# adelacvg/NS2VC

Measured on NVIDIA H100. Metric: denoiser-steps/s, higher is better.
Workload: dtype f32 (3xBF16-split tensor-core contractions, fp32 accumulate)

## Files before the change

### include/ns2vc_b200.h

```cpp
#ifndef NS2VC_B200_H
#define NS2VC_B200_H

#include <stddef.h>
#include <stdint.h>

#ifdef __cplusplus
extern "C" {
#endif

typedef struct ns2vc_unet ns2vc_unet;
typedef void* ns2vc_stream;

#define NS2VC_MAX_LEVELS 8

typedef struct ns2vc_unet_cfg {
  int in_channels;
  int latent_channels;
  int out_channels;
  int n_levels;
  int block_out_channels[NS2VC_MAX_LEVELS];
  int layers_per_block[NS2VC_MAX_LEVELS];
  int down_has_attn[NS2VC_MAX_LEVELS];
  int up_has_attn[NS2VC_MAX_LEVELS];
  int num_heads;
// ... 222 lines not shown
  const float* bias; const float* rowbias; int rowbias_ld;
  const float* res; int res_ld;
  float* out; int out_ld;
  void* out_hi; void* out_lo; int out_split_ld;
  int f16_col0;
  const double* ln_stats; const float* ln_g; int ln_C; float ln_eps;
  double* row_stats; double* stat_sum; double* stat_sq;
  const float* rowmask;
  const int* row_len; int len_shift;
  const float* pre_scale; const float* pre_shift;
  int pre_mode;
  int pre_C;
  int ksplit;
  const double* gn_stats1; const double* gn_stats2; int gn_C1, gn_C2, gn_G; float gn_eps;
  const float* gn_gamma; const float* gn_beta; const float* gn_film; int gn_film_ld;
} ns2vc_check_gemm_args;
typedef struct ns2vc_check_attn_args {
  int B, H, Tq, Tk, dh;
  float scale;
  int v2;
  const float* q; int q_ld; const float* k; int k_ld; const float* v; int v_ld;
  ns2vc_check_split qs, ks, vs;
  int q_c0, k_c0, v_c0;
  int p_split;
  const int* key_len; int key_shift;
  const float* bias;
  float* out; int out_ld;
  void* out_hi; void* out_lo; int out_split_ld;
} ns2vc_check_attn_args;
int ns2vc_check_pack_b(const float* w, int n_rows, int cin_total, int ktaps, int tap, int cin0, int ncin, int n_dst0, int kb0,
                       int geglu_half, const float* cscale, void* w_hi, void* w_lo, int Npad, int nkb_total, ns2vc_stream stream);
int ns2vc_check_gemm(const ns2vc_check_gemm_args* args, char* desc, int desc_len, ns2vc_stream stream);
int ns2vc_check_attention(const ns2vc_check_attn_args* args, char* desc, int desc_len, ns2vc_stream stream);

typedef struct ns2vc_check_prep_args {
  const float* src1; int ld1, C1;
  const float* src2; int ld2, C2;
  int B, T_src, T_dst;
  int row_mul, row_add;
  const int* rowmap;
  int mode;
  const float* scale; const float* shift;
  const double* stats1; const double* stats2;
  const float* gamma; const float* beta; int G; float eps;
  const float* film; int film_ld;
  ns2vc_check_split out, raw;
  const int* row_len; int len_shift;
} ns2vc_check_prep_args;
int ns2vc_check_prep(const ns2vc_check_prep_args* args, char* desc, int desc_len, ns2vc_stream stream);

typedef struct ns2vc_check_ln_args {
  int kind;
  const float* x; int ld, M, C; float eps;
  const float* gamma; const float* beta;
  const float* keep;
  float* y; int y_ld;
  ns2vc_check_split split;
} ns2vc_check_ln_args;
int ns2vc_check_ln(const ns2vc_check_ln_args* args, char* desc, int desc_len, ns2vc_stream stream);

typedef struct ns2vc_check_voc_norm_args {
  const float* x; int B, T, C;
  const float* dw; const float* gamma; const float* beta; float eps;
  const int64_t* len;
  float* out; ns2vc_check_split split;
} ns2vc_check_voc_norm_args;
// ... 57 lines not shown
```

### ns2vc_b200/_lib.py

```python
from __future__ import annotations

import ctypes as C
import os
from typing import Any, Callable, Dict, Optional, Tuple

import torch
import torch.nn as nn

_HERE = os.path.dirname(os.path.abspath(__file__))
LIB_PATH = os.path.join(_HERE, "_C", os.environ.get("NS2VC_LIB_NAME", "libns2vc_b200.so"))

MAX_LEVELS = 8


class UNetCfg(C.Structure):
    _fields_ = [
        ("in_channels", C.c_int), ("latent_channels", C.c_int), ("out_channels", C.c_int), ("n_levels", C.c_int),
        ("block_out_channels", C.c_int * MAX_LEVELS), ("layers_per_block", C.c_int * MAX_LEVELS),
        ("down_has_attn", C.c_int * MAX_LEVELS), ("up_has_attn", C.c_int * MAX_LEVELS),
        ("num_heads", C.c_int), ("cross_attention_dim", C.c_int), ("norm_num_groups", C.c_int), ("norm_eps", C.c_float),
        ("time_scale_shift", C.c_int), ("add_embed_text", C.c_int), ("add_embed_heads", C.c_int),
        ("flip_sin_to_cos", C.c_int), ("freq_shift", C.c_float),
    ]

# ... 108 lines not shown
    "ns2vc_cv_weight_info": (C.c_int, [_P, C.c_int, C.POINTER(C.c_char_p), C.POINTER(C.c_int64), C.POINTER(C.c_int)]),
    "ns2vc_cv_load_weight": (C.c_int, [_P, C.c_char_p, _P, C.POINTER(C.c_int64), C.c_int, _P]),
    "ns2vc_cv_finalize": (C.c_int, [_P, _P]),
    "ns2vc_cv_workspace_bytes": (C.c_int, [_P, C.c_int, C.c_int, C.POINTER(C.c_size_t)]),
    "ns2vc_cv_num_frames": (C.c_int, [C.c_longlong]),
    "ns2vc_cv_extract": (C.c_int, [_P, _P, C.c_longlong, _P, _P, _P, C.c_int, C.c_int, _P, _P]),
    "ns2vc_cv_num_taps": (C.c_int, [_P]),
    "ns2vc_cv_tap_info": (C.c_int, [_P, C.c_int, C.POINTER(C.c_char_p), C.POINTER(C.c_int), C.POINTER(C.c_int)]),
    "ns2vc_cv_set_tap": (C.c_int, [_P, C.c_int, _P]),
    "ns2vc_cv_launch_count": (C.c_int, [_P]),
    "ns2vc_resample_out_length": (C.c_longlong, [C.c_int, C.c_int, C.c_longlong]),
    "ns2vc_resample_table": (C.c_int, [C.c_int, C.c_int, C.POINTER(C.c_int), C.POINTER(C.c_int), C.POINTER(C.c_int), _P]),
    "ns2vc_mel_filterbank": (C.c_int, [_P]),
    "ns2vc_resample_check": (C.c_int, [C.c_int, C.c_int]),
    "ns2vc_resampler_create": (C.c_int, [C.c_int, C.c_int, C.POINTER(_P)]),
    "ns2vc_resampler_destroy": (None, [_P]),
    "ns2vc_resample": (C.c_int, [_P, _P, C.c_longlong, C.c_longlong, _P, _P, C.c_longlong, C.c_longlong, C.c_int, _P]),
    "ns2vc_mel_create": (C.c_int, [_P, _P, C.POINTER(_P)]),
    "ns2vc_mel_destroy": (None, [_P]),
    "ns2vc_log_mel": (C.c_int, [_P, _P, C.c_longlong, C.c_longlong, _P, _P, C.c_int, C.c_int, _P]),
    "ns2vc_stream_sola": (C.c_int, [_P, C.c_longlong, _P, _P, _P, _P, C.c_int, C.c_int, C.c_int, C.c_int, _P]),
    "ns2vc_slice_rms_frames": (C.c_longlong, [C.c_longlong, C.c_int, C.c_int]),
    "ns2vc_slice_rms": (C.c_int, [_P, C.c_longlong, _P, _P, _P, C.c_int, C.c_int, _P]),
    "ns2vc_q_sample": (C.c_int, [_P, _P, C.c_int, _P, _P, _P, _P, C.c_int, _P, _P, _P, C.c_int, C.c_int, C.c_int, C.c_int, _P]),
    "ns2vc_mse_workspace_bytes": (C.c_int, [C.c_int, C.c_int, C.c_int, C.c_int, C.POINTER(C.c_size_t)]),
    "ns2vc_mse_rows": (C.c_int, [_P, _P, C.c_int, _P, _P, C.c_int, C.c_float, _P, _P, _P, C.c_int, C.c_int, C.c_int, C.c_int, _P, _P]),
    "ns2vc_mse_ragged_workspace_bytes": (C.c_int, [C.c_int, C.c_int, C.c_int, C.c_int, C.POINTER(C.c_size_t)]),
    "ns2vc_mse_rows_ragged": (C.c_int, [_P, _P, C.c_int, _P, _P, _P, C.c_int, C.c_float, _P, _P, C.c_int, C.c_int, C.c_int, C.c_int,
                                        _P, _P]),
    "ns2vc_check_pack_b": (C.c_int, [_P, C.c_int, C.c_int, C.c_int, C.c_int, C.c_int, C.c_int, C.c_int, C.c_int, C.c_int, _P, _P, _P,
                                     C.c_int, C.c_int, _P]),
    "ns2vc_check_gemm": (C.c_int, [_P, C.c_char_p, C.c_int, _P]),
    "ns2vc_check_attention": (C.c_int, [_P, C.c_char_p, C.c_int, _P]),
    "ns2vc_check_prep": (C.c_int, [_P, C.c_char_p, C.c_int, _P]),
    "ns2vc_check_ln": (C.c_int, [_P, C.c_char_p, C.c_int, _P]),
    "ns2vc_check_voc_norm": (C.c_int, [_P, C.c_char_p, C.c_int, _P]),
    "ns2vc_check_small_linear": (C.c_int, [_P, C.c_char_p, C.c_int, _P]),
    "ns2vc_check_pool": (C.c_int, [_P, C.c_char_p, C.c_int, _P]),
    "ns2vc_check_nct_split": (C.c_int, [_P, C.c_char_p, C.c_int, _P]),
    "ns2vc_check_cv_conv0": (C.c_int, [_P, C.c_char_p, C.c_int, _P]),
    "ns2vc_check_cv_pos_conv": (C.c_int, [_P, C.c_char_p, C.c_int, _P]),
    "ns2vc_check_istft": (C.c_int, [_P, C.c_char_p, C.c_int, _P]),
}

_lib: Optional[C.CDLL] = None


class Ns2vcError(RuntimeError):
    pass


def lib() -> C.CDLL:
    global _lib
    if _lib is None:
        if not os.path.exists(LIB_PATH):
            raise Ns2vcError(
                f"{LIB_PATH} not found: the ns2vc_b200 CUDA extension is not built "
                "(run ./build.sh or __graft_entry__.build()); there is no CPU fallback.")
        handle = C.CDLL(LIB_PATH)
        for name, (res, args) in SIGNATURES.items():
            fn = getattr(handle, name)
            fn.restype = res
            fn.argtypes = args
        _lib = handle
    return _lib

# ... 130 lines not shown
```

### ns2vc_b200/csrc/attention_v2.cu

```cuda
#include "flash_mma.cuh"
#include "tc_common.cuh"
#include "launch.cuh"
#include <math.h>
#include <cstdlib>

namespace ns2vc {

namespace {

constexpr int kQ = 128, kKeys = 64;
constexpr int kThreadsV2 = 288;

template <int DHP, int PB, bool PF16, bool BIAS> struct ACfg {
  static constexpr int NST = (PB == 128) ? 2 : 3;
  static constexpr int kQBytes = kQ * PB;
  static constexpr int kTBytes = kKeys * PB;
  static constexpr int kStageBytes = 4 * kTBytes;
  static constexpr int kOffQ = 0;
  static constexpr int kOffKV = 2 * kQBytes;
  static constexpr int kOffBar = kOffKV + NST * kStageBytes;
  static constexpr int kOffBias = kOffBar + 256;
  static constexpr int kBiasKeys = (PB == 32) ? 768 : 1024;
  static constexpr int kSmem = kOffBias + (BIAS ? 4 * kBiasKeys : 0) + 1024 ;
  static constexpr int kMinCtas = (PB == 128) ? 1 : (kSmem <= 113 * 1024) ? 2 : 1;
};

template <int DHP, int PB, bool BIAS, bool PF16, bool RAGK = false>
__global__ void __launch_bounds__(kThreadsV2, ACfg<DHP, PB, PF16, BIAS>::kMinCtas) attn_v2_kernel(const __grid_constant__ AttnOp op) {
  using C = ACfg<DHP, PB, PF16, BIAS>;
  constexpr int NST = C::NST;
  extern __shared__ uint8_t smem_raw[];
  const uint32_t raw = smem_u32(smem_raw);
  const uint32_t base = (raw + 1023u) & ~1023u;
  uint8_t* smem = smem_raw + (base - raw);
  const uint32_t bar0 = base + C::kOffBar;
  const uint32_t q_full = bar0;
  auto kv_full = [&](int s) { return bar0 + 8u + 8u * s; };
  auto kv_empty = [&](int s) { return bar0 + 8u + 8u * (NST + s); };

  const int tid = threadIdx.x, warp = tid >> 5, lane = tid & 31;
  const int b = blockIdx.z, h = blockIdx.y, q0 = blockIdx.x * kQ;
  const int dh = op.dh;
  const int ntiles = (op.Tk + kKeys - 1) / kKeys;

  span_begin(op.span);
  const int cta_lin = (blockIdx.z * gridDim.y + blockIdx.y) * gridDim.x + blockIdx.x;
  if (op.trace && tid == 0 && cta_lin < 597) {
    unsigned smid; asm volatile("mov.u32 %0, %%smid;" : "=r"(smid));
    op.trace[256 + 3 * cta_lin] = gtime_ns();
    op.trace[256 + 3 * cta_lin + 2] = smid;
  }
  if (tid == 0) {
    mbar_init(q_full, 1);
    for (int s = 0; s < NST; ++s) { mbar_init(kv_full(s), 1); mbar_init(kv_empty(s), 8); }
    mbar_fence_init();
  }
  if (warp == 0 && lane == 0) {
#pragma unroll
    for (int i = 0; i < 6; ++i) prefetch_tmap(&op.tm[i]);
  }
  pdl_trigger();
  __syncthreads();
  const uint32_t sQ = base + C::kOffQ, sKV = base + C::kOffKV;

  if (warp == 0) {
    if (elect_one()) {
      auto load_kv = [&](int j) {
        const int stage = j % NST;
        const uint32_t dst = sKV + stage * C::kStageBytes;
        mbar_arrive_expect_tx(kv_full(stage), (uint32_t)C::kStageBytes);
        tma_load_3d(dst, &op.tm[2], op.k_c0 + h * dh, j * kKeys, b, kv_full(stage));
        tma_load_3d(dst + C::kTBytes, &op.tm[3], op.k_c0 + h * dh, j * kKeys, b, kv_full(stage));
        tma_load_3d(dst + 2 * C::kTBytes, &op.tm[4], op.v_c0 + h * dh, j * kKeys, b, kv_full(stage));
        tma_load_3d(dst + 3 * C::kTBytes, &op.tm[5], op.v_c0 + h * dh, j * kKeys, b, kv_full(stage));
      };
      pdl_wait();
      int nt = ntiles;
      if constexpr (RAGK) nt = min(ntiles, (((__ldg(op.key_len + b) - 1) >> op.key_shift) + kKeys) / kKeys);
      mbar_arrive_expect_tx(q_full, 2u * C::kQBytes);
      tma_load_3d(sQ, &op.tm[0], op.q_c0 + h * dh, q0, b, q_full);
      tma_load_3d(sQ + C::kQBytes, &op.tm[1], op.q_c0 + h * dh, q0, b, q_full);
      for (int j = 0; j < nt; ++j) {
        if (j >= NST) mbar_wait(kv_empty(j % NST), (uint32_t)(((j / NST) & 1) ^ 1));
        load_kv(j);
      }
    }
  } else {
    float* bias_s = reinterpret_cast<float*>(smem + C::kOffBias);
    const float qscale = op.scale * 1.4426950408889634f;
    pdl_wait();
    int tk = op.Tk, nt = ntiles;
    if constexpr (RAGK) { tk = min(tk, ((__ldg(op.key_len + b) - 1) >> op.key_shift) + 1); nt = (tk + kKeys - 1) / kKeys; }
    if (BIAS) {
      const float* bias = op.bias + (long long)b * op.Tk;
      for (int i = tid - 32; i < ntiles * kKeys; i += 256)
        bias_s[i] = (i < op.Tk) ? __ldg(bias + i) * 1.4426950408889634f : -INFINITY;
      asm volatile("bar.sync 1, 256;" ::: "memory");
    }
    FlashWarp<DHP, PB, PF16> fw;
    const int r0 = 16 * (warp - 1);
    mbar_wait(q_full, 0);
    fw.load_q(sQ, sQ + C::kQBytes, r0, lane);
    for (int j = 0; j < nt; ++j) {
      const int stage = j % NST;
      mbar_wait_quiet(kv_full(stage), (uint32_t)((j / NST) & 1));
      const uint32_t kst = sKV + stage * C::kStageBytes;
      fw.tile(kst, kst + C::kTBytes, kst + 2 * C::kTBytes, kst + 3 * C::kTBytes, BIAS ? bias_s + j * kKeys : nullptr, qscale,
              (RAGK ? tk : op.Tk) - j * kKeys, lane);
      __syncwarp();
      if (lane == 0) mbar_arrive(kv_empty(stage));
    }
    fw.store(op, b, h, q0 + r0, lane);
  }
  __syncthreads();
  span_end(op.span);
  if (op.trace && tid == 0 && cta_lin < 597) op.trace[256 + 3 * cta_lin + 1] = gtime_ns();
}

template <int DHP, int PB, bool BIAS, bool PF16, bool RAGK = false>
int launch_v2b(const AttnOp& op, cudaStream_t st) {
  using C = ACfg<DHP, PB, PF16, BIAS>;
  static bool attr_set = false;
  if (!attr_set) {
    cudaError_t e = cudaFuncSetAttribute(attn_v2_kernel<DHP, PB, BIAS, PF16, RAGK>, cudaFuncAttributeMaxDynamicSharedMemorySize, C::kSmem);
    if (e != cudaSuccess) { set_error("attention v2: cannot set %d B dynamic smem: %s", C::kSmem, cudaGetErrorString(e)); return -2; }
    cudaFuncSetAttribute(attn_v2_kernel<DHP, PB, BIAS, PF16, RAGK>, cudaFuncAttributePreferredSharedMemoryCarveout, (int)cudaSharedmemCarveoutMaxShared);
    if (getenv("NS2VC_DEBUG")) {
      int nb = 0;
      cudaOccupancyMaxActiveBlocksPerMultiprocessor(&nb, attn_v2_kernel<DHP, PB, BIAS, PF16, RAGK>, kThreadsV2, (size_t)C::kSmem);
      fprintf(stderr, "ns2vc: attn_v2<%d,%d,bias=%d,f16=%d> smem %d B, planned %d CTAs/SM, occupancy API says %d\n", DHP, PB, (int)BIAS, (int)PF16, C::kSmem, C::kMinCtas, nb);
    }
    attr_set = true;
  }
  dim3 grid(ceil_div(op.Tq, kQ), op.H, op.B);
  cudaError_t e = launch_k(attn_v2_kernel<DHP, PB, BIAS, PF16, RAGK>, grid, dim3(kThreadsV2), (size_t)C::kSmem, st, op);
  if (e != cudaSuccess) { set_error("attention v2 launch failed: %s", cudaGetErrorString(e)); return -2; }
  return 0;
}
bool p_fp16() { return attention_v2_p_fp16(); }
template <int DHP, int PB>
int launch_v2(const AttnOp& op, cudaStream_t st) {
  if (op.key_len) {
    if (op.bias) { set_error("attention v2: per-entry key counts take no additive bias"); return -1; }
    return (p_fp16() && !op.p_split) ? launch_v2b<DHP, PB, false, true, true>(op, st) : launch_v2b<DHP, PB, false, false, true>(op, st);
  }
  if (op.bias) {
    if (ceil_div(op.Tk, kKeys) * kKeys > ACfg<DHP, PB, true, true>::kBiasKeys) { set_error("attention v2: %d biased keys exceed the staged-bias capacity", op.Tk); return -1; }
    return (p_fp16() && !op.p_split) ? launch_v2b<DHP, PB, true, true>(op, st) : launch_v2b<DHP, PB, true, false>(op, st);
  }
  return (p_fp16() && !op.p_split) ? launch_v2b<DHP, PB, false, true>(op, st) : launch_v2b<DHP, PB, false, false>(op, st);
}

int natural_pb(int dh) { return dh == 16 ? 32 : dh == 32 ? 64 : 128; }

}

bool attention_v2_p_fp16() {
  static int v = -1;
  if (v < 0) { const char* e = getenv("NS2VC_ATTN_P"); v = (e && e[0] == 's') ? 0 : 1; }
  return v == 1;
}

bool attention_v2_supported(int dh, int Tk, bool biased) {
  if (!(dh == 16 || dh == 32 || dh == 48 || dh == 64)) return false;
  return !biased || ceil_div(Tk, kKeys) * kKeys <= (dh == 16 ? 768 : 1024);
}

int encode_attn_tmaps(AttnOp& op) {
  op.pb = natural_pb(op.dh);
  const int bc = op.pb / 2;
  int rc = 0;
  if ((rc = encode_tmap_rows(&op.tm[0], op.qs.hi, op.qs.C, op.qs.T, op.B, op.qs.ld, bc, kQ, op.pb))) return rc;
  if ((rc = encode_tmap_rows(&op.tm[1], op.qs.lo, op.qs.C, op.qs.T, op.B, op.qs.ld, bc, kQ, op.pb))) return rc;
  if ((rc = encode_tmap_rows(&op.tm[2], op.ks.hi, op.ks.C, op.ks.T, op.B, op.ks.ld, bc, kKeys, op.pb))) return rc;
  if ((rc = encode_tmap_rows(&op.tm[3], op.ks.lo, op.ks.C, op.ks.T, op.B, op.ks.ld, bc, kKeys, op.pb))) return rc;
  if ((rc = encode_tmap_rows(&op.tm[4], op.vs.hi, op.vs.C, op.vs.T, op.B, op.vs.ld, bc, kKeys, op.pb))) return rc;
  if ((rc = encode_tmap_rows(&op.tm[5], op.vs.lo, op.vs.C, op.vs.T, op.B, op.vs.ld, bc, kKeys, op.pb))) return rc;
  return 0;
}

int launch_attention_v2(const AttnOp& op, cudaStream_t st) {
  if (op.Tk <= 0 || op.Tq <= 0) { set_error("attention: empty sequence"); return -1; }
  if (op.qs.T != op.Tq || op.ks.T != op.Tk || op.vs.T != op.Tk) { set_error("attention v2: split buffer / sequence length mismatch"); return -1; }
  const int dh = op.dh;
  if (op.pb == 128) {
    if (dh == 48) return launch_v2<48, 128>(op, st);
    if (dh == 64) return launch_v2<64, 128>(op, st);
  } else if (op.pb == 64 && dh == 32) {
    return launch_v2<32, 64>(op, st);
  } else if (op.pb == 32 && dh == 16) {
    return launch_v2<16, 32>(op, st);
  }
  set_error("attention v2: unsupported head dim %d / box %d", dh, op.pb);
  return -1;
// ... 4 lines not shown
```

### ns2vc_b200/csrc/common.cuh

```cuda
#pragma once
#include <cuda_runtime.h>
#include <cuda_bf16.h>
#include <stdint.h>
#include <stddef.h>

namespace ns2vc {

void set_error(const char* fmt, ...);
const char* get_error();

#define NS_CHECK_CUDA(expr)                                                                    \
  do {                                                                                         \
    cudaError_t _e = (expr);                                                                   \
    if (_e != cudaSuccess) {                                                                   \
      ns2vc::set_error("%s:%d CUDA error %s: %s", __FILE__, __LINE__, cudaGetErrorName(_e),    \
                       cudaGetErrorString(_e));                                                \
      return -2;                                                                               \
    }                                                                                          \
  } while (0)

#define NS_REQUIRE(cond, ...)                                                                  \
  do {                                                                                         \
    if (!(cond)) {                                                                             \
      ns2vc::set_error(__VA_ARGS__);                                                           \
// ... 151 lines not shown
  const float* gamma; const float* beta;
  const float* keep;
  float* y; int y_ld;
  SplitBuf split;
};
int launch_ln_split(const LnOp& op, cudaStream_t st);

struct AttnOp {
  const float* q; int q_ld;
  const float* k; int k_ld;
  const float* v; int v_ld;
  const float* bias;
  float* out; int out_ld;
  __nv_bfloat16* out_hi;
  __nv_bfloat16* out_lo;
  int out_split_ld;
  int B, H, Tq, Tk, dh;
  float scale;
  unsigned long long* span;
  unsigned long long* trace;
  SplitBuf qs, ks, vs;
  int q_c0, k_c0, v_c0;
  int v2;
  int pb;
  const int* key_len;
  int key_shift;
  int p_split;
  TMap tm[6];
};
int launch_attention(const AttnOp& op, cudaStream_t st, bool simt_debug);
int launch_attention_v2(const AttnOp& op, cudaStream_t st);
bool attention_v2_supported(int dh, int Tk, bool biased);
bool attention_v2_p_fp16();
int encode_attn_tmaps(AttnOp& op);
int encode_tmap_rows(TMap* out, const __nv_bfloat16* base, int C, int T, int B, int ld, int box_c, int box_rows, int swizzle_bytes);
int encode_tmap_any(TMap* out, const void* base, int elem_bytes, int C, int T, int B, int ld, int box_c, int box_rows, int swizzle_bytes,
                    long long bpitch = 0);

int launch_ln_apply(const LnOp& op, cudaStream_t st);

struct TokensOp {
  const float* x; long long bstride; int B, C, T;
  float* out; int ld;
  const float* rowbias;
  const float* keep;
};
int launch_nct_to_tokens(const TokensOp& op, cudaStream_t st);
struct NctSplitOp {
  const float* x; long long bstride; int B, C, T;
  SplitBuf out;
  const int* row_len;
  const void* warm; long long warm_bytes;
};
int launch_nct_to_split(const NctSplitOp& op, cudaStream_t st);

enum LinIn : int { LIN_RAW = 0, LIN_SILU = 1, LIN_SINUSOID = 2 };
struct LinOp {
  const float* x; int x_ld; int M; int K;
  const float* W; const float* bias; int N;
  const float* add; int add_ld;
  int add_rows;
  float* out; int out_ld;
  int in_mode; int flip_sin_to_cos; float freq_shift;
  int out_silu;
};
int launch_small_linear(const LinOp& op, cudaStream_t st);
// ... 105 lines not shown
```

### ns2vc_b200/csrc/flash_mma.cuh

```cuda
#pragma once
#include "gemm_common.cuh"
#include <math.h>

namespace ns2vc {

template <int PB>
__device__ __forceinline__ uint32_t swz(uint32_t a) { return a ^ (((a >> 7) & (uint32_t)(PB / 16 - 1)) << 4); }

__device__ __forceinline__ float ex2f(float x) { float y; asm("ex2.approx.ftz.f32 %0, %1;" : "=f"(y) : "f"(x)); return y; }

__device__ __forceinline__ void ldsm_x4(uint32_t a, uint32_t* r) {
  asm volatile("ldmatrix.sync.aligned.m8n8.x4.shared.b16 {%0, %1, %2, %3}, [%4];" : "=r"(r[0]), "=r"(r[1]), "=r"(r[2]), "=r"(r[3]) : "r"(a));
}
__device__ __forceinline__ void ldsm_x4_t(uint32_t a, uint32_t* r) {
  asm volatile("ldmatrix.sync.aligned.m8n8.x4.trans.shared.b16 {%0, %1, %2, %3}, [%4];" : "=r"(r[0]), "=r"(r[1]), "=r"(r[2]), "=r"(r[3]) : "r"(a));
}
#define NS2VC_MMA(name, ty)                                                                                                      \
  __device__ __forceinline__ void name(float* c, const uint32_t* a, uint32_t b0, uint32_t b1) {                               \
    asm volatile("mma.sync.aligned.m16n8k16.row.col.f32." ty "." ty ".f32 {%0, %1, %2, %3}, {%4, %5, %6, %7}, {%8, %9}, {%0, %1, %2, %3};" \
                 : "+f"(c[0]), "+f"(c[1]), "+f"(c[2]), "+f"(c[3]) : "r"(a[0]), "r"(a[1]), "r"(a[2]), "r"(a[3]), "r"(b0), "r"(b1)); }
NS2VC_MMA(mma_bf16, "bf16")
NS2VC_MMA(mma_f16, "f16")
#undef NS2VC_MMA

template <int DHP, int PB, bool PF16>
struct FlashWarp {
  static constexpr int KS = DHP / 16;
  static constexpr int NO = DHP / 8;
  uint32_t qh[KS][4], ql[KS][4];
  float o[NO][4];
  float m[2], l[2];

  __device__ __forceinline__ void load_q(uint32_t sqh, uint32_t sql, int r0, int lane) {
    const uint32_t off = (uint32_t)((r0 + (lane & 7) + 8 * ((lane >> 3) & 1)) * PB + 16 * (lane >> 4));
#pragma unroll
    for (int k = 0; k < KS; ++k) { ldsm_x4(swz<PB>(sqh + off + 32 * k), qh[k]); ldsm_x4(swz<PB>(sql + off + 32 * k), ql[k]); }
#pragma unroll
    for (int n = 0; n < NO; ++n) o[n][0] = o[n][1] = o[n][2] = o[n][3] = 0.f;
    m[0] = m[1] = -INFINITY;
    l[0] = l[1] = 0.f;
  }

  __device__ __forceinline__ void tile(uint32_t skh, uint32_t skl, uint32_t svh, uint32_t svl, const float* bias, float qs, int nvalid, int lane) {
    float s[8][4];
#pragma unroll
    for (int n = 0; n < 8; ++n) s[n][0] = s[n][1] = s[n][2] = s[n][3] = 0.f;
    const uint32_t koff = (uint32_t)(((lane & 7) + 8 * (lane >> 4)) * PB + 16 * ((lane >> 3) & 1));
#pragma unroll
    for (int k = 0; k < KS; ++k) {
#pragma unroll
      for (int np = 0; np < 4; ++np) {
        uint32_t kh[4], kl[4];
        const uint32_t a = (uint32_t)(16 * np * PB) + koff + 32 * k;
        ldsm_x4(swz<PB>(skh + a), kh);
        ldsm_x4(swz<PB>(skl + a), kl);
        mma_bf16(s[2 * np], qh[k], kh[0], kh[1]);
        mma_bf16(s[2 * np], ql[k], kh[0], kh[1]);
        mma_bf16(s[2 * np], qh[k], kl[0], kl[1]);
        mma_bf16(s[2 * np + 1], qh[k], kh[2], kh[3]);
        mma_bf16(s[2 * np + 1], ql[k], kh[2], kh[3]);
        mma_bf16(s[2 * np + 1], qh[k], kl[2], kl[3]);
      }
    }
    const int t = lane & 3;
    float mx[2] = {-INFINITY, -INFINITY};
#pragma unroll
    for (int n = 0; n < 8; ++n)
#pragma unroll
      for (int e = 0; e < 4; ++e) {
        const int key = 8 * n + 2 * t + (e & 1);
        float v = s[n][e] * qs;
        if (bias) v += bias[key];
        else if (key >= nvalid) v = -INFINITY;
        s[n][e] = v;
        mx[e >> 1] = fmaxf(mx[e >> 1], v);
      }
    float corr[2];
#pragma unroll
    for (int i = 0; i < 2; ++i) {
      mx[i] = fmaxf(mx[i], __shfl_xor_sync(0xffffffffu, mx[i], 1));
      mx[i] = fmaxf(mx[i], __shfl_xor_sync(0xffffffffu, mx[i], 2));
      const float mn = fmaxf(m[i], mx[i]);
      corr[i] = ex2f(m[i] - mn);
      m[i] = mn;
      l[i] *= corr[i];
    }
#pragma unroll
    for (int n = 0; n < NO; ++n)
#pragma unroll
      for (int e = 0; e < 4; ++e) o[n][e] *= corr[e >> 1];
    const uint32_t voff = (uint32_t)(((lane & 7) + 8 * ((lane >> 3) & 1)) * PB + 16 * (lane >> 4));
#pragma unroll
    for (int kk = 0; kk < 4; ++kk) {
      uint32_t ph[4], pl[4];
#pragma unroll
      for (int u = 0; u < 4; ++u) {
        float* sv = s[2 * kk + (u >> 1)] + 2 * (u & 1);
        const float p0 = ex2f(sv[0] - m[u & 1]), p1 = ex2f(sv[1] - m[u & 1]);
        if (PF16) {
          ph[u] = pack_f16x2(p0, p1);
          l[u & 1] += f16lo_to_f32(ph[u]) + f16hi_to_f32(ph[u]);
        } else {
          split2(p0, p1, ph[u], pl[u]);
          l[u & 1] += p0 + p1;
        }
      }
#pragma unroll
      for (int dp = 0; dp < NO / 2; ++dp) {
        uint32_t vh[4], vl[4];
        const uint32_t a = (uint32_t)(16 * kk * PB) + voff + 32 * dp;
        ldsm_x4_t(swz<PB>(svh + a), vh);
        ldsm_x4_t(swz<PB>(svl + a), vl);
        if (PF16) {
          mma_f16(o[2 * dp], ph, vh[0], vh[1]);
          mma_f16(o[2 * dp], ph, vl[0], vl[1]);
          mma_f16(o[2 * dp + 1], ph, vh[2], vh[3]);
          mma_f16(o[2 * dp + 1], ph, vl[2], vl[3]);
        } else {
          mma_bf16(o[2 * dp], ph, vh[0], vh[1]);
          mma_bf16(o[2 * dp], pl, vh[0], vh[1]);
          mma_bf16(o[2 * dp], ph, vl[0], vl[1]);
          mma_bf16(o[2 * dp + 1], ph, vh[2], vh[3]);
          mma_bf16(o[2 * dp + 1], pl, vh[2], vh[3]);
          mma_bf16(o[2 * dp + 1], ph, vl[2], vl[3]);
        }
      }
    }
  }

  __device__ __forceinline__ void store(const AttnOp& op, int b, int h, int q0, int lane) {
    const int g = lane >> 2, t = lane & 3;
#pragma unroll
    for (int i = 0; i < 2; ++i) {
      l[i] += __shfl_xor_sync(0xffffffffu, l[i], 1);
      l[i] += __shfl_xor_sync(0xffffffffu, l[i], 2);
    }
#pragma unroll
    for (int i = 0; i < 2; ++i) {
      const int q = q0 + g + 8 * i;
      if (q >= op.Tq) continue;
      const float inv = 1.0f / l[i];
      const long long orow = (long long)b * op.Tq + q;
#pragma unroll
      for (int n = 0; n < NO; ++n) {
        const int d = 8 * n + 2 * t;
        if (d >= op.dh) continue;
        const float v0 = o[n][2 * i] * inv, v1 = o[n][2 * i + 1] * inv;
        const long long of = orow * op.out_ld + h * op.dh + d, os = orow * op.out_split_ld + h * op.dh + d;
        if (op.out && d + 1 < op.dh && ((of | (long long)(reinterpret_cast<uintptr_t>(op.out) >> 2)) & 1) == 0) {
          *reinterpret_cast<float2*>(op.out + of) = make_float2(v0, v1);
        } else if (op.out) {
          op.out[of] = v0;
          if (d + 1 < op.dh) op.out[of + 1] = v1;
        }
        if (op.out_hi && d + 1 < op.dh &&
            ((os | (long long)(reinterpret_cast<uintptr_t>(op.out_hi) >> 1) | (long long)(reinterpret_cast<uintptr_t>(op.out_lo) >> 1)) & 1) == 0) {
          uint32_t hi, lo;
          split2(v0, v1, hi, lo);
          *reinterpret_cast<uint32_t*>(op.out_hi + os) = hi;
          *reinterpret_cast<uint32_t*>(op.out_lo + os) = lo;
        } else if (op.out_hi) {
#pragma unroll
          for (int e = 0; e < 2; ++e) {
            if (d + e >= op.dh) break;
            const float v = e ? v1 : v0;
            const __nv_bfloat16 hi = __float2bfloat16_rn(v);
            op.out_hi[os + e] = hi;
            op.out_lo[os + e] = __float2bfloat16_rn(v - __bfloat162float(hi));
          }
        }
      }
    }
  }
};

}
```

### ns2vc_b200/csrc/kernel_check.cu

```cuda
#include "engine_host.cuh"
#include "../../include/ns2vc_b200.h"

#include <cstdio>
#include <vector>

namespace ns2vc {
namespace {

SplitBuf to_split(const ns2vc_check_split& s) {
  SplitBuf b{};
  b.hi = (__nv_bfloat16*)s.hi; b.lo = (__nv_bfloat16*)s.lo; b.T = s.T; b.C = s.C; b.ld = s.ld; b.bpitch = s.bpitch;
  return b;
}

template <class... A> void report(char* desc, int desc_len, const char* fmt, A... args) {
  if (desc && desc_len > 0) snprintf(desc, (size_t)desc_len, fmt, args...);
}

}
}

using namespace ns2vc;

extern "C" {
// ... 100 lines not shown
int ns2vc_check_attention(const ns2vc_check_attn_args* a, char* desc, int desc_len, ns2vc_stream stream) {
  NS_REQUIRE(a, "check_attention: null argument");
  NS_REQUIRE(a->B >= 1 && a->H >= 1 && a->dh >= 1, "check_attention: bad sizes B=%d H=%d dh=%d", a->B, a->H, a->dh);
  NS_REQUIRE(a->out || (a->out_hi && a->out_lo), "check_attention: no output");
  AttnOp op; memset(&op, 0, sizeof(op));
  op.B = a->B; op.H = a->H; op.Tq = a->Tq; op.Tk = a->Tk; op.dh = a->dh; op.scale = a->scale;
  op.bias = a->bias;
  op.out = a->out; op.out_ld = a->out_ld;
  op.out_hi = (__nv_bfloat16*)a->out_hi; op.out_lo = (__nv_bfloat16*)a->out_lo; op.out_split_ld = a->out_split_ld;
  cudaStream_t st = (cudaStream_t)stream;
  if (a->v2) {
    NS_REQUIRE(a->qs.hi && a->qs.lo && a->ks.hi && a->ks.lo && a->vs.hi && a->vs.lo, "check_attention: v2 needs split q / k / v");
    op.v2 = 1;
    op.qs = to_split(a->qs); op.ks = to_split(a->ks); op.vs = to_split(a->vs);
    op.q_c0 = a->q_c0; op.k_c0 = a->k_c0; op.v_c0 = a->v_c0;
    op.key_len = a->key_len; op.key_shift = a->key_shift; op.p_split = a->p_split;
    int rc = encode_attn_tmaps(op);
    if (!rc) rc = launch_attention_v2(op, st);
    if (rc) return rc;
    const bool pf16 = attention_v2_p_fp16() && !op.p_split;
    report(desc, desc_len, "attn_v2<%d,PB=%d,BIAS=%d,PF16=%d,RAGK=%d>", op.dh, op.pb, op.bias ? 1 : 0, pf16 ? 1 : 0, op.key_len ? 1 : 0);
    return 0;
  }
  NS_REQUIRE(a->q && a->k && a->v, "check_attention: v1 needs fp32 q / k / v");
  NS_REQUIRE(!a->key_len, "check_attention: per-entry key counts are a v2 feature");
  op.q = a->q; op.q_ld = a->q_ld; op.k = a->k; op.k_ld = a->k_ld; op.v = a->v; op.v_ld = a->v_ld;
  const int rc = launch_attention(op, st, false);
  if (rc) return rc;
  const int dhp = a->dh <= 16 ? 16 : a->dh <= 32 ? 32 : a->dh <= 48 ? 48 : 64;
  report(desc, desc_len, "attn_tc<%d>", dhp);
  return 0;
}

int ns2vc_check_prep(const ns2vc_check_prep_args* a, char* desc, int desc_len, ns2vc_stream stream) {
  NS_REQUIRE(a, "check_prep: null argument");
  NS_REQUIRE(a->B >= 1 && a->T_src >= 1 && a->T_dst >= 1 && a->C1 >= 1 && a->C2 >= 0 && a->src1 && (a->C2 == 0 || a->src2),
             "check_prep: bad sizes B=%d T=%d->%d C=%d+%d", a->B, a->T_src, a->T_dst, a->C1, a->C2);
  NS_REQUIRE(a->out.hi && a->out.lo, "check_prep: no output");
  NS_REQUIRE(a->mode >= PREP_RAW && a->mode <= PREP_AFFINE_SILU, "check_prep: mode %d", a->mode);
  PrepOp p; memset(&p, 0, sizeof(p));
  p.src1 = a->src1; p.ld1 = a->ld1; p.C1 = a->C1; p.src2 = a->src2; p.ld2 = a->ld2; p.C2 = a->C2;
  p.B = a->B; p.T_src = a->T_src; p.T_dst = a->T_dst;
  p.row_mul = a->row_mul; p.row_add = a->row_add; p.rowmap = a->rowmap; p.mode = a->mode;
  p.out = to_split(a->out);
  if (a->raw.hi) p.raw = to_split(a->raw);
  p.row_len = a->row_len; p.len_shift = a->len_shift;
  if (a->mode != PREP_RAW) {
    if (a->scale) {
      NS_REQUIRE(a->shift, "check_prep: scale without shift");
      p.scale = a->scale; p.shift = a->shift;
    } else {
      NS_REQUIRE(a->stats1 && (a->C2 == 0 || a->stats2) && a->gamma && a->beta && a->G >= 1, "check_prep: GroupNorm without its sums or weights");
      set_group_norm(p, a->B, a->stats1, a->C1, a->C2 ? a->stats2 : nullptr, a->C2, a->T_src, a->G, a->eps, a->gamma, a->beta, a->film,
                     a->film_ld);
    }
  }
  const int rc = launch_prep_split(p, (cudaStream_t)stream);
  if (rc) return rc;
  report(desc, desc_len, "prep_split<RAG=%d>", p.row_len ? 1 : 0);
  return 0;
}

int ns2vc_check_ln(const ns2vc_check_ln_args* a, char* desc, int desc_len, ns2vc_stream stream) {
  NS_REQUIRE(a && a->x && a->gamma && a->beta, "check_ln: null argument");
  NS_REQUIRE(a->M >= 1 && a->C >= 1 && a->ld >= a->C, "check_ln: bad sizes M=%d C=%d ld=%d", a->M, a->C, a->ld);
  LnOp op{a->x, a->ld, a->M, a->C, a->eps, a->gamma, a->beta, a->keep, a->y, a->y_ld, to_split(a->split)};
// ... 163 lines not shown
```

Baseline: 1804.

## Add wgmma warpgroup core for attention v2 and make it the default

```diff
diff --git a/include/ns2vc_b200.h b/include/ns2vc_b200.h
--- a/include/ns2vc_b200.h
+++ b/include/ns2vc_b200.h
@@ -278,6 +278,8 @@
                        int geglu_half, const float* cscale, void* w_hi, void* w_lo, int Npad, int nkb_total, ns2vc_stream stream);
 int ns2vc_check_gemm(const ns2vc_check_gemm_args* args, char* desc, int desc_len, ns2vc_stream stream);
 int ns2vc_check_attention(const ns2vc_check_attn_args* args, char* desc, int desc_len, ns2vc_stream stream);
+int ns2vc_attention_set_core(int core);
+int ns2vc_attention_core(int dh, int pf16);
 
 typedef struct ns2vc_check_prep_args {
   const float* src1; int ld1, C1;
diff --git a/ns2vc_b200/_lib.py b/ns2vc_b200/_lib.py
--- a/ns2vc_b200/_lib.py
+++ b/ns2vc_b200/_lib.py
@@ -164,6 +164,8 @@
                                      C.c_int, C.c_int, _P]),
     "ns2vc_check_gemm": (C.c_int, [_P, C.c_char_p, C.c_int, _P]),
     "ns2vc_check_attention": (C.c_int, [_P, C.c_char_p, C.c_int, _P]),
+    "ns2vc_attention_set_core": (C.c_int, [C.c_int]),
+    "ns2vc_attention_core": (C.c_int, [C.c_int, C.c_int]),
     "ns2vc_check_prep": (C.c_int, [_P, C.c_char_p, C.c_int, _P]),
     "ns2vc_check_ln": (C.c_int, [_P, C.c_char_p, C.c_int, _P]),
     "ns2vc_check_voc_norm": (C.c_int, [_P, C.c_char_p, C.c_int, _P]),
diff --git a/ns2vc_b200/csrc/attention_v2.cu b/ns2vc_b200/csrc/attention_v2.cu
--- a/ns2vc_b200/csrc/attention_v2.cu
+++ b/ns2vc_b200/csrc/attention_v2.cu
@@ -1,4 +1,4 @@
-#include "flash_mma.cuh"
+#include "flash_wgmma.cuh"
 #include "tc_common.cuh"
 #include "launch.cuh"
 #include <math.h>
@@ -25,7 +25,7 @@
   static constexpr int kMinCtas = (PB == 128) ? 1 : (kSmem <= 113 * 1024) ? 2 : 1;
 };
 
-template <int DHP, int PB, bool BIAS, bool PF16, bool RAGK = false>
+template <int DHP, int PB, bool BIAS, bool PF16, bool RAGK, bool WG>
 __global__ void __launch_bounds__(kThreadsV2, ACfg<DHP, PB, PF16, BIAS>::kMinCtas) attn_v2_kernel(const __grid_constant__ AttnOp op) {
   using C = ACfg<DHP, PB, PF16, BIAS>;
   constexpr int NST = C::NST;
@@ -55,7 +55,7 @@
     for (int s = 0; s < NST; ++s) { mbar_init(kv_full(s), 1); mbar_init(kv_empty(s), 8); }
     mbar_fence_init();
   }
-  if (warp == 0 && lane == 0) {
+  if (warp == 8 && lane == 0) {
 #pragma unroll
     for (int i = 0; i < 6; ++i) prefetch_tmap(&op.tm[i]);
   }
@@ -63,7 +63,7 @@
   __syncthreads();
   const uint32_t sQ = base + C::kOffQ, sKV = base + C::kOffKV;
 
-  if (warp == 0) {
+  if (warp == 8) {
     if (elect_one()) {
       auto load_kv = [&](int j) {
         const int stage = j % NST;
@@ -93,20 +93,24 @@
     if constexpr (RAGK) { tk = min(tk, ((__ldg(op.key_len + b) - 1) >> op.key_shift) + 1); nt = (tk + kKeys - 1) / kKeys; }
     if (BIAS) {
       const float* bias = op.bias + (long long)b * op.Tk;
-      for (int i = tid - 32; i < ntiles * kKeys; i += 256)
+      for (int i = tid; i < ntiles * kKeys; i += 256)
         bias_s[i] = (i < op.Tk) ? __ldg(bias + i) * 1.4426950408889634f : -INFINITY;
       asm volatile("bar.sync 1, 256;" ::: "memory");
     }
-    FlashWarp<DHP, PB, PF16> fw;
-    const int r0 = 16 * (warp - 1);
+    const int r0 = 16 * warp;
+    std::conditional_t<WG, FlashWG<DHP, PB, PF16>, FlashWarp<DHP, PB, PF16>> fw;
+    const uint32_t sqh = sQ + (r0 & ~63) * PB;
     mbar_wait(q_full, 0);
-    fw.load_q(sQ, sQ + C::kQBytes, r0, lane);
+    if constexpr (WG) fw.init();
+    else fw.load_q(sQ, sQ + C::kQBytes, r0, lane);
     for (int j = 0; j < nt; ++j) {
       const int stage = j % NST;
       mbar_wait_quiet(kv_full(stage), (uint32_t)((j / NST) & 1));
       const uint32_t kst = sKV + stage * C::kStageBytes;
-      fw.tile(kst, kst + C::kTBytes, kst + 2 * C::kTBytes, kst + 3 * C::kTBytes, BIAS ? bias_s + j * kKeys : nullptr, qscale,
-              (RAGK ? tk : op.Tk) - j * kKeys, lane);
+      const float* bj = BIAS ? bias_s + j * kKeys : nullptr;
+      const int nvalid = (RAGK ? tk : op.Tk) - j * kKeys;
+      if constexpr (WG) fw.tile(sqh, sqh + C::kQBytes, kst, kst + C::kTBytes, kst + 2 * C::kTBytes, kst + 3 * C::kTBytes, bj, qscale, nvalid, lane);
+      else fw.tile(kst, kst + C::kTBytes, kst + 2 * C::kTBytes, kst + 3 * C::kTBytes, bj, qscale, nvalid, lane);
       __syncwarp();
       if (lane == 0) mbar_arrive(kv_empty(stage));
     }
@@ -117,25 +121,35 @@
   if (op.trace && tid == 0 && cta_lin < 597) op.trace[256 + 3 * cta_lin + 1] = gtime_ns();
 }
 
+template <int DHP, int PB, bool BIAS, bool PF16, bool RAGK, bool WG>
+int launch_v2c(const AttnOp& op, cudaStream_t st) {
+  using C = ACfg<DHP, PB, PF16, BIAS>;
+  auto kern = attn_v2_kernel<DHP, PB, BIAS, PF16, RAGK, WG>;
+  static bool attr_set = false;
+  if (!attr_set) {
+    cudaError_t e = cudaFuncSetAttribute(kern, cudaFuncAttributeMaxDynamicSharedMemorySize, C::kSmem);
+    if (e != cudaSuccess) { set_error("attention v2: cannot set %d B dynamic smem: %s", C::kSmem, cudaGetErrorString(e)); return -2; }
+    cudaFuncSetAttribute(kern, cudaFuncAttributePreferredSharedMemoryCarveout, (int)cudaSharedmemCarveoutMaxShared);
+    if (getenv("NS2VC_DEBUG")) {
+      int nb = 0;
+      cudaOccupancyMaxActiveBlocksPerMultiprocessor(&nb, kern, kThreadsV2, (size_t)C::kSmem);
+      fprintf(stderr, "ns2vc: attn_v2<%d,%d,bias=%d,f16=%d,wg=%d> smem %d B, planned %d CTAs/SM, occupancy API says %d\n", DHP, PB,
+              (int)BIAS, (int)PF16, (int)WG, C::kSmem, C::kMinCtas, nb);
+    }
+    attr_set = true;
+  }
+  dim3 grid(ceil_div(op.Tq, kQ), op.H, op.B);
+  cudaError_t e = launch_k(kern, grid, dim3(kThreadsV2), (size_t)C::kSmem, st, op);
+  if (e != cudaSuccess) { set_error("attention v2 launch failed: %s", cudaGetErrorString(e)); return -2; }
+  return 0;
+}
+
+int g_core = 0;
+bool core_wg() { return g_core != 1; }
+
 template <int DHP, int PB, bool BIAS, bool PF16, bool RAGK = false>
 int launch_v2b(const AttnOp& op, cudaStream_t st) {
-  using C = ACfg<DHP, PB, PF16, BIAS>;
-  static bool attr_set = false;
-  if (!attr_set) {
-    cudaError_t e = cudaFuncSetAttribute(attn_v2_kernel<DHP, PB, BIAS, PF16, RAGK>, cudaFuncAttributeMaxDynamicSharedMemorySize, C::kSmem);
-    if (e != cudaSuccess) { set_error("attention v2: cannot set %d B dynamic smem: %s", C::kSmem, cudaGetErrorString(e)); return -2; }
-    cudaFuncSetAttribute(attn_v2_kernel<DHP, PB, BIAS, PF16, RAGK>, cudaFuncAttributePreferredSharedMemoryCarveout, (int)cudaSharedmemCarveoutMaxShared);
-    if (getenv("NS2VC_DEBUG")) {
-      int nb = 0;
-      cudaOccupancyMaxActiveBlocksPerMultiprocessor(&nb, attn_v2_kernel<DHP, PB, BIAS, PF16, RAGK>, kThreadsV2, (size_t)C::kSmem);
-      fprintf(stderr, "ns2vc: attn_v2<%d,%d,bias=%d,f16=%d> smem %d B, planned %d CTAs/SM, occupancy API says %d\n", DHP, PB, (int)BIAS, (int)PF16, C::kSmem, C::kMinCtas, nb);
-    }
-    attr_set = true;
-  }
-  dim3 grid(ceil_div(op.Tq, kQ), op.H, op.B);
-  cudaError_t e = launch_k(attn_v2_kernel<DHP, PB, BIAS, PF16, RAGK>, grid, dim3(kThreadsV2), (size_t)C::kSmem, st, op);
-  if (e != cudaSuccess) { set_error("attention v2 launch failed: %s", cudaGetErrorString(e)); return -2; }
-  return 0;
+  return core_wg() ? launch_v2c<DHP, PB, BIAS, PF16, RAGK, true>(op, st) : launch_v2c<DHP, PB, BIAS, PF16, RAGK, false>(op, st);
 }
 bool p_fp16() { return attention_v2_p_fp16(); }
 template <int DHP, int PB>
@@ -160,6 +174,14 @@
   if (v < 0) { const char* e = getenv("NS2VC_ATTN_P"); v = (e && e[0] == 's') ? 0 : 1; }
   return v == 1;
 }
+
+int attention_v2_set_core(int core) {
+  if (core < 0 || core > 2) { set_error("attention v2: core %d is not 0 (measured choice), 1 (mma.sync warps) or 2 (wgmma warpgroups)", core); return -1; }
+  g_core = core;
+  return 0;
+}
+
+int attention_v2_core(int dh, bool pf16) { (void)dh; (void)pf16; return core_wg() ? 2 : 1; }
 
 bool attention_v2_supported(int dh, int Tk, bool biased) {
   if (!(dh == 16 || dh == 32 || dh == 48 || dh == 64)) return false;
diff --git a/ns2vc_b200/csrc/common.cuh b/ns2vc_b200/csrc/common.cuh
--- a/ns2vc_b200/csrc/common.cuh
+++ b/ns2vc_b200/csrc/common.cuh
@@ -207,6 +207,8 @@
 int launch_attention_v2(const AttnOp& op, cudaStream_t st);
 bool attention_v2_supported(int dh, int Tk, bool biased);
 bool attention_v2_p_fp16();
+int attention_v2_set_core(int core);
+int attention_v2_core(int dh, bool pf16);
 int encode_attn_tmaps(AttnOp& op);
 int encode_tmap_rows(TMap* out, const __nv_bfloat16* base, int C, int T, int B, int ld, int box_c, int box_rows, int swizzle_bytes);
 int encode_tmap_any(TMap* out, const void* base, int elem_bytes, int C, int T, int B, int ld, int box_c, int box_rows, int swizzle_bytes,
diff --git a/ns2vc_b200/csrc/flash_mma.cuh b/ns2vc_b200/csrc/flash_mma.cuh
--- a/ns2vc_b200/csrc/flash_mma.cuh
+++ b/ns2vc_b200/csrc/flash_mma.cuh
@@ -22,6 +22,100 @@
 NS2VC_MMA(mma_bf16, "bf16")
 NS2VC_MMA(mma_f16, "f16")
 #undef NS2VC_MMA
+
+template <int NO>
+__device__ __forceinline__ void flash_rescale(float (&s)[8][4], float (&o)[NO][4], float (&m)[2], float (&l)[2], const float* bias,
+                                              float qs, int nvalid, int lane) {
+  const int t = lane & 3;
+  float mx[2] = {-INFINITY, -INFINITY};
+#pragma unroll
+  for (int n = 0; n < 8; ++n)
+#pragma unroll
+    for (int e = 0; e < 4; ++e) {
+      const int key = 8 * n + 2 * t + (e & 1);
+      float v = s[n][e] * qs;
+      if (bias) v += bias[key];
+      else if (key >= nvalid) v = -INFINITY;
+      s[n][e] = v;
+      mx[e >> 1] = fmaxf(mx[e >> 1], v);
+    }
+  float corr[2];
+#pragma unroll
+  for (int i = 0; i < 2; ++i) {
+    mx[i] = fmaxf(mx[i], __shfl_xor_sync(0xffffffffu, mx[i], 1));
+    mx[i] = fmaxf(mx[i], __shfl_xor_sync(0xffffffffu, mx[i], 2));
+    const float mn = fmaxf(m[i], mx[i]);
+    corr[i] = ex2f(m[i] - mn);
+    m[i] = mn;
+    l[i] *= corr[i];
+  }
+#pragma unroll
+  for (int n = 0; n < NO; ++n)
+#pragma unroll
+    for (int e = 0; e < 4; ++e) o[n][e] *= corr[e >> 1];
+}
+
+template <bool PF16>
+__device__ __forceinline__ void flash_weights(const float (&s)[8][4], const float (&m)[2], float (&l)[2], int kk, uint32_t* ph, uint32_t* pl) {
+#pragma unroll
+  for (int u = 0; u < 4; ++u) {
+    const float* sv = s[2 * kk + (u >> 1)] + 2 * (u & 1);
+    const float p0 = ex2f(sv[0] - m[u & 1]), p1 = ex2f(sv[1] - m[u & 1]);
+    if (PF16) {
+      ph[u] = pack_f16x2(p0, p1);
+      l[u & 1] += f16lo_to_f32(ph[u]) + f16hi_to_f32(ph[u]);
+    } else {
+      split2(p0, p1, ph[u], pl[u]);
+      l[u & 1] += p0 + p1;
+    }
+  }
+}
+
+template <int NO>
+__device__ __forceinline__ void flash_store(const float (&o)[NO][4], float (&l)[2], const AttnOp& op, int b, int h, int q0, int lane) {
+  const int g = lane >> 2, t = lane & 3;
+#pragma unroll
+  for (int i = 0; i < 2; ++i) {
+    l[i] += __shfl_xor_sync(0xffffffffu, l[i], 1);
+    l[i] += __shfl_xor_sync(0xffffffffu, l[i], 2);
+  }
+#pragma unroll
+  for (int i = 0; i < 2; ++i) {
+    const int q = q0 + g + 8 * i;
+    if (q >= op.Tq) continue;
+    const float inv = 1.0f / l[i];
+    const long long orow = (long long)b * op.Tq + q;
+#pragma unroll
+    for (int n = 0; n < NO; ++n) {
+      const int d = 8 * n + 2 * t;
+      if (d >= op.dh) continue;
+      const float v0 = o[n][2 * i] * inv, v1 = o[n][2 * i + 1] * inv;
+      const long long of = orow * op.out_ld + h * op.dh + d, os = orow * op.out_split_ld + h * op.dh + d;
+      if (op.out && d + 1 < op.dh && ((of | (long long)(reinterpret_cast<uintptr_t>(op.out) >> 2)) & 1) == 0) {
+        *reinterpret_cast<float2*>(op.out + of) = make_float2(v0, v1);
+      } else if (op.out) {
+        op.out[of] = v0;
+        if (d + 1 < op.dh) op.out[of + 1] = v1;
+      }
+      if (op.out_hi && d + 1 < op.dh &&
+          ((os | (long long)(reinterpret_cast<uintptr_t>(op.out_hi) >> 1) | (long long)(reinterpret_cast<uintptr_t>(op.out_lo) >> 1)) & 1) == 0) {
+        uint32_t hi, lo;
+        split2(v0, v1, hi, lo);
+        *reinterpret_cast<uint32_t*>(op.out_hi + os) = hi;
+        *reinterpret_cast<uint32_t*>(op.out_lo + os) = lo;
+      } else if (op.out_hi) {
+#pragma unroll
+        for (int e = 0; e < 2; ++e) {
+          if (d + e >= op.dh) break;
+          const float v = e ? v1 : v0;
+          const __nv_bfloat16 hi = __float2bfloat16_rn(v);
+          op.out_hi[os + e] = hi;
+          op.out_lo[os + e] = __float2bfloat16_rn(v - __bfloat162float(hi));
+        }
+      }
+    }
+  }
+}
 
 template <int DHP, int PB, bool PF16>
 struct FlashWarp {
@@ -62,49 +156,12 @@
         mma_bf16(s[2 * np + 1], qh[k], kl[2], kl[3]);
       }
     }
-    const int t = lane & 3;
-    float mx[2] = {-INFINITY, -INFINITY};
-#pragma unroll
-    for (int n = 0; n < 8; ++n)
-#pragma unroll
-      for (int e = 0; e < 4; ++e) {
-        const int key = 8 * n + 2 * t + (e & 1);
-        float v = s[n][e] * qs;
-        if (bias) v += bias[key];
-        else if (key >= nvalid) v = -INFINITY;
-        s[n][e] = v;
-        mx[e >> 1] = fmaxf(mx[e >> 1], v);
-      }
-    float corr[2];
-#pragma unroll
-    for (int i = 0; i < 2; ++i) {
-      mx[i] = fmaxf(mx[i], __shfl_xor_sync(0xffffffffu, mx[i], 1));
-      mx[i] = fmaxf(mx[i], __shfl_xor_sync(0xffffffffu, mx[i], 2));
-      const float mn = fmaxf(m[i], mx[i]);
-      corr[i] = ex2f(m[i] - mn);
-      m[i] = mn;
-      l[i] *= corr[i];
-    }
-#pragma unroll
-    for (int n = 0; n < NO; ++n)
-#pragma unroll
-      for (int e = 0; e < 4; ++e) o[n][e] *= corr[e >> 1];
+    flash_rescale<NO>(s, o, m, l, bias, qs, nvalid, lane);
     const uint32_t voff = (uint32_t)(((lane & 7) + 8 * ((lane >> 3) & 1)) * PB + 16 * (lane >> 4));
 #pragma unroll
     for (int kk = 0; kk < 4; ++kk) {
       uint32_t ph[4], pl[4];
-#pragma unroll
-      for (int u = 0; u < 4; ++u) {
-        float* sv = s[2 * kk + (u >> 1)] + 2 * (u & 1);
-        const float p0 = ex2f(sv[0] - m[u & 1]), p1 = ex2f(sv[1] - m[u & 1]);
-        if (PF16) {
-          ph[u] = pack_f16x2(p0, p1);
-          l[u & 1] += f16lo_to_f32(ph[u]) + f16hi_to_f32(ph[u]);
-        } else {
-          split2(p0, p1, ph[u], pl[u]);
-          l[u & 1] += p0 + p1;
-        }
-      }
+      flash_weights<PF16>(s, m, l, kk, ph, pl);
 #pragma unroll
       for (int dp = 0; dp < NO / 2; ++dp) {
         uint32_t vh[4], vl[4];
@@ -128,50 +185,7 @@
     }
   }
 
-  __device__ __forceinline__ void store(const AttnOp& op, int b, int h, int q0, int lane) {
-    const int g = lane >> 2, t = lane & 3;
-#pragma unroll
-    for (int i = 0; i < 2; ++i) {
-      l[i] += __shfl_xor_sync(0xffffffffu, l[i], 1);
-      l[i] += __shfl_xor_sync(0xffffffffu, l[i], 2);
-    }
-#pragma unroll
-    for (int i = 0; i < 2; ++i) {
-      const int q = q0 + g + 8 * i;
-      if (q >= op.Tq) continue;
-      const float inv = 1.0f / l[i];
-      const long long orow = (long long)b * op.Tq + q;
-#pragma unroll
-      for (int n = 0; n < NO; ++n) {
-        const int d = 8 * n + 2 * t;
-        if (d >= op.dh) continue;
-        const float v0 = o[n][2 * i] * inv, v1 = o[n][2 * i + 1] * inv;
-        const long long of = orow * op.out_ld + h * op.dh + d, os = orow * op.out_split_ld + h * op.dh + d;
-        if (op.out && d + 1 < op.dh && ((of | (long long)(reinterpret_cast<uintptr_t>(op.out) >> 2)) & 1) == 0) {
-          *reinterpret_cast<float2*>(op.out + of) = make_float2(v0, v1);
-        } else if (op.out) {
-          op.out[of] = v0;
-          if (d + 1 < op.dh) op.out[of + 1] = v1;
-        }
-        if (op.out_hi && d + 1 < op.dh &&
-            ((os | (long long)(reinterpret_cast<uintptr_t>(op.out_hi) >> 1) | (long long)(reinterpret_cast<uintptr_t>(op.out_lo) >> 1)) & 1) == 0) {
-          uint32_t hi, lo;
-          split2(v0, v1, hi, lo);
-          *reinterpret_cast<uint32_t*>(op.out_hi + os) = hi;
-          *reinterpret_cast<uint32_t*>(op.out_lo + os) = lo;
-        } else if (op.out_hi) {
-#pragma unroll
-          for (int e = 0; e < 2; ++e) {
-            if (d + e >= op.dh) break;
-            const float v = e ? v1 : v0;
-            const __nv_bfloat16 hi = __float2bfloat16_rn(v);
-            op.out_hi[os + e] = hi;
-            op.out_lo[os + e] = __float2bfloat16_rn(v - __bfloat162float(hi));
-          }
-        }
-      }
-    }
-  }
+  __device__ __forceinline__ void store(const AttnOp& op, int b, int h, int q0, int lane) { flash_store<NO>(o, l, op, b, h, q0, lane); }
 };
 
 }
diff --git a/ns2vc_b200/csrc/flash_wgmma.cuh b/ns2vc_b200/csrc/flash_wgmma.cuh
--- /dev/null
+++ b/ns2vc_b200/csrc/flash_wgmma.cuh
@@ -0,0 +1,115 @@
+#pragma once
+#include "flash_mma.cuh"
+#include "tc_common.cuh"
+
+namespace ns2vc {
+
+template <int PB>
+__device__ __forceinline__ uint64_t wg_desc_rows(uint32_t saddr) {
+  constexpr uint64_t mode = PB == 128 ? 1 : PB == 64 ? 2 : 3;
+  return (uint64_t)((saddr & 0x3FFFFu) >> 4) | (1ull << 16) | ((uint64_t)((8 * PB) >> 4) << 32) | (mode << 62);
+}
+
+template <int N, bool F16>
+__device__ __forceinline__ void wgmma_rs(float* d, const uint32_t* a, uint64_t bdesc);
+#define NS2VC_D8(i) "+f"(d[i]), "+f"(d[i + 1]), "+f"(d[i + 2]), "+f"(d[i + 3]), "+f"(d[i + 4]), "+f"(d[i + 5]), "+f"(d[i + 6]), "+f"(d[i + 7])
+#define NS2VC_A4 "r"(a[0]), "r"(a[1]), "r"(a[2]), "r"(a[3])
+template <>
+__device__ __forceinline__ void wgmma_rs<16, true>(float* d, const uint32_t* a, uint64_t bdesc) {
+  asm volatile("{\n\t.reg .pred p;\n\tsetp.ne.b32 p, %13, 0;\n\twgmma.mma_async.sync.aligned.m64n16k16.f32.f16.f16 "
+               "{%0,%1,%2,%3,%4,%5,%6,%7}, "
+               "{%8,%9,%10,%11}, %12, p, 1, 1, 1;\n\t}" : NS2VC_D8(0) : NS2VC_A4, "l"(bdesc), "r"(1));
+}
+template <>
+__device__ __forceinline__ void wgmma_rs<16, false>(float* d, const uint32_t* a, uint64_t bdesc) {
+  asm volatile("{\n\t.reg .pred p;\n\tsetp.ne.b32 p, %13, 0;\n\twgmma.mma_async.sync.aligned.m64n16k16.f32.bf16.bf16 "
+               "{%0,%1,%2,%3,%4,%5,%6,%7}, "
+               "{%8,%9,%10,%11}, %12, p, 1, 1, 1;\n\t}" : NS2VC_D8(0) : NS2VC_A4, "l"(bdesc), "r"(1));
+}
+template <>
+__device__ __forceinline__ void wgmma_rs<32, true>(float* d, const uint32_t* a, uint64_t bdesc) {
+  asm volatile("{\n\t.reg .pred p;\n\tsetp.ne.b32 p, %21, 0;\n\twgmma.mma_async.sync.aligned.m64n32k16.f32.f16.f16 "
+               "{%0,%1,%2,%3,%4,%5,%6,%7,%8,%9,%10,%11,%12,%13,%14,%15}, "
+               "{%16,%17,%18,%19}, %20, p, 1, 1, 1;\n\t}" : NS2VC_D8(0), NS2VC_D8(8) : NS2VC_A4, "l"(bdesc), "r"(1));
+}
+template <>
+__device__ __forceinline__ void wgmma_rs<32, false>(float* d, const uint32_t* a, uint64_t bdesc) {
+  asm volatile("{\n\t.reg .pred p;\n\tsetp.ne.b32 p, %21, 0;\n\twgmma.mma_async.sync.aligned.m64n32k16.f32.bf16.bf16 "
+               "{%0,%1,%2,%3,%4,%5,%6,%7,%8,%9,%10,%11,%12,%13,%14,%15}, "
+               "{%16,%17,%18,%19}, %20, p, 1, 1, 1;\n\t}" : NS2VC_D8(0), NS2VC_D8(8) : NS2VC_A4, "l"(bdesc), "r"(1));
+}
+template <>
+__device__ __forceinline__ void wgmma_rs<48, true>(float* d, const uint32_t* a, uint64_t bdesc) {
+  asm volatile("{\n\t.reg .pred p;\n\tsetp.ne.b32 p, %29, 0;\n\twgmma.mma_async.sync.aligned.m64n48k16.f32.f16.f16 "
+               "{%0,%1,%2,%3,%4,%5,%6,%7,%8,%9,%10,%11,%12,%13,%14,%15,%16,%17,%18,%19,%20,%21,%22,%23}, "
+               "{%24,%25,%26,%27}, %28, p, 1, 1, 1;\n\t}" : NS2VC_D8(0), NS2VC_D8(8), NS2VC_D8(16) : NS2VC_A4, "l"(bdesc), "r"(1));
+}
+template <>
+__device__ __forceinline__ void wgmma_rs<48, false>(float* d, const uint32_t* a, uint64_t bdesc) {
+  asm volatile("{\n\t.reg .pred p;\n\tsetp.ne.b32 p, %29, 0;\n\twgmma.mma_async.sync.aligned.m64n48k16.f32.bf16.bf16 "
+               "{%0,%1,%2,%3,%4,%5,%6,%7,%8,%9,%10,%11,%12,%13,%14,%15,%16,%17,%18,%19,%20,%21,%22,%23}, "
+               "{%24,%25,%26,%27}, %28, p, 1, 1, 1;\n\t}" : NS2VC_D8(0), NS2VC_D8(8), NS2VC_D8(16) : NS2VC_A4, "l"(bdesc), "r"(1));
+}
+template <>
+__device__ __forceinline__ void wgmma_rs<64, true>(float* d, const uint32_t* a, uint64_t bdesc) {
+  asm volatile("{\n\t.reg .pred p;\n\tsetp.ne.b32 p, %37, 0;\n\twgmma.mma_async.sync.aligned.m64n64k16.f32.f16.f16 "
+               "{%0,%1,%2,%3,%4,%5,%6,%7,%8,%9,%10,%11,%12,%13,%14,%15,%16,%17,%18,%19,%20,%21,%22,%23,%24,%25,%26,%27,%28,%29,%30,%31}, "
+               "{%32,%33,%34,%35}, %36, p, 1, 1, 1;\n\t}" : NS2VC_D8(0), NS2VC_D8(8), NS2VC_D8(16), NS2VC_D8(24) : NS2VC_A4, "l"(bdesc), "r"(1));
+}
+template <>
+__device__ __forceinline__ void wgmma_rs<64, false>(float* d, const uint32_t* a, uint64_t bdesc) {
+  asm volatile("{\n\t.reg .pred p;\n\tsetp.ne.b32 p, %37, 0;\n\twgmma.mma_async.sync.aligned.m64n64k16.f32.bf16.bf16 "
+               "{%0,%1,%2,%3,%4,%5,%6,%7,%8,%9,%10,%11,%12,%13,%14,%15,%16,%17,%18,%19,%20,%21,%22,%23,%24,%25,%26,%27,%28,%29,%30,%31}, "
+               "{%32,%33,%34,%35}, %36, p, 1, 1, 1;\n\t}" : NS2VC_D8(0), NS2VC_D8(8), NS2VC_D8(16), NS2VC_D8(24) : NS2VC_A4, "l"(bdesc), "r"(1));
+}
+#undef NS2VC_A4
+#undef NS2VC_D8
+
+template <int DHP, int PB, bool PF16>
+struct FlashWG {
+  static constexpr int KS = DHP / 16;
+  static constexpr int NO = DHP / 8;
+  float o[NO][4];
+  float m[2], l[2];
+
+  __device__ __forceinline__ void init() {
+#pragma unroll
+    for (int n = 0; n < NO; ++n) o[n][0] = o[n][1] = o[n][2] = o[n][3] = 0.f;
+    m[0] = m[1] = -INFINITY;
+    l[0] = l[1] = 0.f;
+  }
+
+  __device__ __forceinline__ void tile(uint32_t sqh, uint32_t sql, uint32_t skh, uint32_t skl, uint32_t svh, uint32_t svl,
+                                       const float* bias, float qs, int nvalid, int lane) {
+    float s[8][4];
+#pragma unroll
+    for (int n = 0; n < 8; ++n) s[n][0] = s[n][1] = s[n][2] = s[n][3] = 0.f;
+    wgmma_fence();
+#pragma unroll
+    for (int k = 0; k < KS; ++k) {
+      const uint64_t kh = wg_desc_rows<PB>(skh + 32 * k);
+      wgmma_bf16<64>(&s[0][0], wg_desc_rows<PB>(sqh + 32 * k), kh);
+      wgmma_bf16<64>(&s[0][0], wg_desc_rows<PB>(sql + 32 * k), kh);
+      wgmma_bf16<64>(&s[0][0], wg_desc_rows<PB>(sqh + 32 * k), wg_desc_rows<PB>(skl + 32 * k));
+    }
+    wgmma_commit();
+    wgmma_wait<0>();
+    flash_rescale<NO>(s, o, m, l, bias, qs, nvalid, lane);
+    uint32_t ph[4][4], pl[4][4];
+#pragma unroll
+    for (int kk = 0; kk < 4; ++kk) flash_weights<PF16>(s, m, l, kk, ph[kk], pl[kk]);
+    wgmma_fence();
+#pragma unroll
+    for (int kk = 0; kk < 4; ++kk) {
+      const uint64_t vh = wg_desc_rows<PB>(svh + 16 * kk * PB), vl = wg_desc_rows<PB>(svl + 16 * kk * PB);
+      wgmma_rs<DHP, PF16>(&o[0][0], ph[kk], vh);
+      if (!PF16) wgmma_rs<DHP, PF16>(&o[0][0], pl[kk], vh);
+      wgmma_rs<DHP, PF16>(&o[0][0], ph[kk], vl);
+    }
+    wgmma_commit();
+    wgmma_wait<0>();
+  }
+
+  __device__ __forceinline__ void store(const AttnOp& op, int b, int h, int q0, int lane) { flash_store<NO>(o, l, op, b, h, q0, lane); }
+};
+}
diff --git a/ns2vc_b200/csrc/kernel_check.cu b/ns2vc_b200/csrc/kernel_check.cu
--- a/ns2vc_b200/csrc/kernel_check.cu
+++ b/ns2vc_b200/csrc/kernel_check.cu
@@ -156,6 +156,9 @@
   return 0;
 }
 
+int ns2vc_attention_set_core(int core) { return attention_v2_set_core(core); }
+int ns2vc_attention_core(int dh, int pf16) { return attention_v2_core(dh, pf16 != 0); }
+
 int ns2vc_check_prep(const ns2vc_check_prep_args* a, char* desc, int desc_len, ns2vc_stream stream) {
   NS_REQUIRE(a, "check_prep: null argument");
   NS_REQUIRE(a->B >= 1 && a->T_src >= 1 && a->T_dst >= 1 && a->C1 >= 1 && a->C2 >= 0 && a->src1 && (a->C2 == 0 || a->src2),
```

Result: faster. 1848 (median of 6 runs) (+2.4%).
